# worxli/ORB_SLAM

Hardware: AMD Instinct MI355X
Metric: frames/sec ORB extract+match (640x480, 1000 kp) (higher is better)
Workload: dtype u8

## Files before the change

### orb_slam_amd/__init__.py

```python
import ctypes
import os
from pathlib import Path

import numpy as np

_PKG = Path(__file__).resolve().parent
LIB_PATH = Path(os.environ.get("ORBX_LIBRARY", _PKG / "liborbx.so"))

ORBX_OK = 0
ERRORS = {-1: "ORBX_ERR_ARG", -2: "ORBX_ERR_HIP", -3: "ORBX_ERR_CAPACITY",
          -4: "ORBX_ERR_UNSUPPORTED", -5: "ORBX_ERR_NOMEM", -6: "ORBX_ERR_NOT_POSDEF"}

KEYPOINT = np.dtype([("x", "<f4"), ("y", "<f4"), ("size", "<f4"), ("angle", "<f4"),
                     ("response", "<f4"), ("octave", "<i4"), ("class_id", "<i4")])
assert KEYPOINT.itemsize == 28


class OrbxError(RuntimeError):
    def __init__(self, code, where):
        super().__init__(f"{where}: {ERRORS.get(code, code)}")
        self.code = code


class FrameView(ctypes.Structure):
# ... 242 lines not shown
        "orbx_vocab_n_words": ([vp], i),
        "orbx_vocab_transform": ([vp, vp, i, vp, i, vp, vp, vp, vp, vp, ip, vp, vp, vp, ip], i),
        "orbx_dev_compute_bow": ([vp, vp, i, i, i], i),
        "orbx_dev_read_bow": ([vp, i, i, vp, vp, vp, vp, vp, ip, vp, vp, vp, ip], i),
        "orbx_dev_search_by_bow": ([vp, i, i, vp, f, i, vp, i, vp], i),
        "orbx_dev_search_by_bow_kf": ([vp, i, vp, i, vp, vp, f, i, vp, i, vp], i),
        "orbx_dev_search_for_triangulation": ([vp, i, vp, i, vp, vp, vp, vp, i, i, vp, i, vp], i),
        "orbx_undistort_keypoints": ([vp, i, vp, vp, vp, vp], i),
        "orbx_compute_image_bounds": ([i, i, vp, vp, vp], i),
        "orbx_dev_undistort": ([vp, i, i, vp, vp], i),
        "orbx_pose_optimization": ([vp, vp, ip, vp], i),
        "orbx_pose_optimization_batch": ([vp, i, vp, vp, vp], i),
        "orbx_pose_stage": ([vp, i, vp], i),
        "orbx_pose_run": ([vp], i),
        "orbx_pose_fetch": ([vp, vp, vp, vp], i),
        "orbx_version": ([], ctypes.c_char_p),
        "orbx_abi_version": ([], i),
        "orbx_lba_set_workgroups": ([vp, i], i),
        "orbx_lba_get_workgroups": ([vp], i),
        "orbx_lba_last_workgroups": ([vp], i),
        "orbx_debug_lba_split": ([vp, i, i, i, i], i),
        "orbx_debug_describe_patch": ([vp, i, i, i, i, vp], i),
        "orbx_debug_level0_direct": ([vp], i),
        "orbx_pose_set_exact": ([vp, i], i),
        "orbx_pose_get_exact": ([vp], i),
        "orbx_dev_set_image_bounds": ([vp, vp], i),
        "orbx_set_launch_mode": ([vp, i], i),
        "orbx_get_launch_mode": ([vp], i),
        "orbx_host_alloc": ([sz, ctypes.POINTER(vp)], i),
        "orbx_host_free": ([vp], None),
        "orbx_dev_upload_async": ([vp, i, i, vp, i, i, sz], i),
        "orbx_dev_download_async": ([vp, i, i, vp, vp, vp, vp, vp], i),
        "orbx_describe_levels": ([i, f, i, i, i, i, vp, i], i),
        "orbx_init_models": ([vp, vp], i),
        "orbx_init_models_batch": ([vp, i, vp], i),
        "orbx_dev_init_models": ([vp, i, i, i, f, i, vp], i),
        "orbx_dev_read_init_models": ([vp, i, vp], i),
        "orbx_init_reconstruct": ([vp, vp], i),
        "orbx_init_reconstruct_batch": ([vp, i, vp], i),
        "orbx_dev_init_reconstruct": ([vp, i, i, i, vp, f, f, i], i),
        "orbx_dev_read_init_reconstruct": ([vp, i, vp, ip], i),
        "orbx_triangulate_matches": ([vp, vp, i, vp, i, vp, vp, vp, vp, vp, vp, vp, vp], i),
        "orbx_create_new_map_points": ([vp, vp, vp, i, vp, vp, vp, i, i, vp, vp, vp, vp, vp, vp], i),
        "orbx_dev_create_new_map_points": ([vp, i, vp, vp, i, vp, vp, vp, vp, i, i, vp, vp, vp, vp, vp, vp, i], i),
    }
    for name, (args, res) in sigs.items():
# ... 150 lines not shown
        nm, n1 = ctypes.c_int(0), ctypes.c_int(0)
        _check(lib().orbx_dev_read_matches(self._h, slot, _ptr(m), self.nfeatures, ctypes.byref(nm),
                                           ctypes.byref(n1)), "orbx_dev_read_matches")
        return m, nm.value

    def level(self, slot, level, blurred=False, cap=4 << 20):
        buf = np.zeros(cap, np.uint8)
        pw, ph = ctypes.c_int(0), ctypes.c_int(0)
        _check(lib().orbx_dev_read_level(self._h, slot, level, int(blurred), _ptr(buf), cap,
                                         ctypes.byref(pw), ctypes.byref(ph)), "orbx_dev_read_level")
        return buf[:pw.value * ph.value].reshape(ph.value, pw.value).copy()

    def describe_patch(self, slot, level, x, y):
        out = np.zeros((37, 37), np.uint8)
        _check(lib().orbx_debug_describe_patch(self._h, slot, level, x, y, _ptr(out)), "orbx_debug_describe_patch")
        return out

    def level0_direct(self):
        r = lib().orbx_debug_level0_direct(self._h)
        if r < 0:
            raise OrbxError(r, "orbx_debug_level0_direct")
        return bool(r)

    def timing(self, enable=True, only=None):
        _check(lib().orbx_dev_kernel_time_select(self._h, only.encode() if only else None), "timing")
        _check(lib().orbx_dev_kernel_time_enable(self._h, int(enable)), "timing")

    def kernel_time(self, name):
        avg, tot = ctypes.c_double(0), ctypes.c_double(0)
        n = lib().orbx_dev_kernel_time(self._h, name.encode(), ctypes.byref(avg), ctypes.byref(tot))
        if n < 0:
            raise OrbxError(n, "orbx_dev_kernel_time")
        return n, avg.value, tot.value

    def pose_optimization(self, frames):
        from .synth_pose import PoseStats
        arr = (type(frames[0]) * len(frames))(*frames)
        n = np.zeros(len(frames), np.int32)
        st = (PoseStats * len(frames))()
        _check(lib().orbx_pose_optimization_batch(self._h, len(frames), arr, _ptr(n), st),
               "orbx_pose_optimization_batch")
        for k in range(len(frames)):
            frames[k].Tcw = arr[k].Tcw
        return n, list(st)

    def pose_stage(self, frames):
# ... 238 lines not shown
```

### orb_slam_amd/csrc/orbx_extract.hip

```cpp
#include <algorithm>
#include <type_traits>

#include "orbx_device.h"
#include "orbx_internal.h"

namespace orbx {

constexpr size_t kRetainLds = 128 * 1024;
constexpr int kRetainCellCap = 512;
constexpr int kSplitMinFrames = 16;
constexpr size_t kResizeLds = 96 * 1024;

__constant__ __attribute__((aligned(4))) int8_t c_pattern[256][4] = {
#include "orbx_pattern.inc"
};

#ifdef ORBX_FAST_PROFILE
__device__ unsigned long long g_fast_prof[16];
__device__ inline unsigned long long fp_stamp()
{
    unsigned long long t;
    asm volatile("s_memtime %0\n\ts_waitcnt lgkmcnt(0)" : "=s"(t)::"memory");
    return t;
}
#define FP_T0() unsigned long long _ft = fp_stamp()
#define FP_MARK(k)                                                                  \
    do {                                                                            \
        const unsigned long long _n = fp_stamp();                                   \
        if (threadIdx.x == 0) atomicAdd(&g_fast_prof[k], _n - _ft);                 \
        _ft = _n;                                                                   \
    } while (0)
#define FP_ADD(k, v) atomicAdd(&g_fast_prof[k], (unsigned long long)(v))
extern "C" int orbx_debug_fast_prof(unsigned long long* out)
{
    return hipMemcpyFromSymbol(out, HIP_SYMBOL(g_fast_prof), sizeof(unsigned long long) * 16) == hipSuccess ? 0 : -2;
}
#else
#define FP_T0()
#define FP_MARK(k)
#define FP_ADD(k, v)
#endif

struct ExtractArgs {
    const LevelGeom* levels;
    const CellGeom* cells;
    const ResizeCol* res_cols;
    const ResizeRow* res_rows;
    const int* umax;
    const uint8_t* frames;
    uint8_t* pyr_raw;
    uint8_t* pyr_blur;
    uint32_t* cell_lists;
    int32_t* cell_count;
    uint32_t* level_keys;
    int32_t* level_count;
    orbx_keypoint* out_kps;
    uint8_t* out_desc;
    int32_t* out_n;
// ... 19 lines not shown
    int stride;
};
static_assert(kEdge % 16 == 0, "the direct level 0 keeps the padded level's 16-byte alignment");
__device__ __forceinline__ LevelSrc level_src(const ExtractArgs& a, int f, int level, long long off, int stride)
{
    if (a.l0_direct && level == 0)
        return {a.frames + ((long long)(a.first_slot + f) * a.w * a.h - (long long)kEdge * a.w - kEdge), a.w};
    return {a.pyr_raw + (size_t)f * a.frame_pyr_bytes + off, stride};
}

template <class T>
__device__ __forceinline__ T cget(const T* p, int i)
{
#if defined(__HIP_DEVICE_COMPILE__)
    return ((const __attribute__((address_space(4))) T*)p)[i];
#else
    return p[i];
#endif
}

__device__ inline uint8_t sat_u8(int v) { return (uint8_t)min(max(v, 0), 255); }
__device__ inline int sat_s16(int v) { return min(max(v, -32768), 32767); }

struct RowWalk {
    int r, q, dr, dq, nq;
    __device__ RowWalk(int start, int stride, int n_q) : nq(n_q)
    {
        r = start / n_q;
        q = start - r * n_q;
        dr = stride / n_q;
        dq = stride - dr * n_q;
    }
    __device__ void next()
    {
        r += dr;
        q += dq;
        if (q >= nq) {
            q -= nq;
            r++;
        }
    }
};


template <int kBatch, typename T, typename Load>
__device__ inline void stage_to_lds(T* dst, int n, int tid, int nthr, Load load)
{
    for (int u0 = 0; u0 < n; u0 += kBatch * nthr) {
        T v[kBatch];
#pragma unroll
        for (int k = 0; k < kBatch; k++) v[k] = load(min(u0 + k * nthr + tid, n - 1));
#pragma unroll
        for (int k = 0; k < kBatch; k++) dst[min(u0 + k * nthr + tid, n - 1)] = v[k];
    }
}

constexpr int kPyrRows = 8;
constexpr int kPyr0Shift = (16 - kEdge % 16) % 16;

__global__ __launch_bounds__(256) void k_pyr_level0(ExtractArgs a, int q_lo, int nint)
{
    const int f = blockIdx.y;
    const LevelGeom L = cget(a.levels, 0);
    const int qpr = L.stride >> 4, nstrips = (L.ph + kPyrRows - 1) / kPyrRows;
    const int nbord = qpr - nint;
    int idx = blockIdx.x * blockDim.x + threadIdx.x;
    const uint8_t* src = a.frames + (size_t)(a.first_slot + f) * a.w * a.h;
// ... 515 lines not shown
                *reinterpret_cast<uint4*>(out + (size_t)(kEdge + r) * stride + 16 * q) =
                    *reinterpret_cast<const uint4*>(dst + (r - c0) * stride + 16 * q);
            }
            for (int i = tid; i < 2 * kEdge * n16; i += T) {
                const int k = i / n16, q = i - k * n16;
                const int py = k < kEdge ? k : L.h + k;
                const int r = reflect101(py - kEdge, L.h);
                if (r >= pl.x && r < pl.y)
                    *reinterpret_cast<uint4*>(out + (size_t)py * stride + 16 * q) =
                        *reinterpret_cast<const uint4*>(dst + (r - c0) * stride + 16 * q);
            }
        }
        CASC_MARK(l, 3);
        if (l > 0) {
            tcol += L.w;
            trow += max(0, nrows);
        }
        sc0 = c0;
        sstride = stride;
    }
}

typedef _Float16 orbx_h2 __attribute__((ext_vector_type(2)));
typedef unsigned short orbx_u16x2 __attribute__((ext_vector_type(2)));
__device__ inline orbx_h2 h2_min3(orbx_h2 a, orbx_h2 b, orbx_h2 c)
{
    return __builtin_elementwise_minimum(__builtin_elementwise_minimum(a, b), c);
}
__device__ inline orbx_h2 h2_max3(orbx_h2 a, orbx_h2 b, orbx_h2 c)
{
    return __builtin_elementwise_maximum(__builtin_elementwise_maximum(a, b), c);
}
__device__ inline void fast_arc2(const uint8_t* t, int pa, int pb, int pitch, int& Sa, int& Sb)
{
    const int off[16] = {3 * pitch,      1 + 3 * pitch, 2 + 2 * pitch,  3 + pitch,
                         3,              3 - pitch,     2 - 2 * pitch,  1 - 3 * pitch,
                         -3 * pitch,     -1 - 3 * pitch, -2 - 2 * pitch, -3 - pitch,
                         -3,             -3 + pitch,    -2 + 2 * pitch, -1 + 3 * pitch};
    const int o = 3 * pitch + 3;
    int ba = pa - o, bb = pb - o;
    asm("" : "+v"(ba), "+v"(bb));
    const uint8_t* ta = t + ba;
    const uint8_t* tb = t + bb;
    auto pair = [&](int k) {
        orbx_u16x2 pv;
        pv.x = ta[k];
        pv.y = tb[k];
        return __builtin_bit_cast(uint32_t, pv) | 0x64006400u;
    };
    const orbx_h2 v = __builtin_bit_cast(orbx_h2, pair(o));
    orbx_h2 d[16];
#pragma unroll
    for (int k = 0; k < 16; k++) {
        const uint32_t w = pair(off[k] + o);
        d[k] = v - __builtin_bit_cast(orbx_h2, w);
    }
    orbx_h2 lo3[16], hi3[16];
#pragma unroll
    for (int k = 0; k < 16; k++) {
        lo3[k] = h2_min3(d[k], d[(k + 1) & 15], d[(k + 2) & 15]);
        hi3[k] = h2_max3(d[k], d[(k + 1) & 15], d[(k + 2) & 15]);
    }
    orbx_h2 m9[16], x9[16];
#pragma unroll
    for (int k = 0; k < 16; k++) {
        m9[k] = h2_min3(lo3[k], lo3[(k + 3) & 15], lo3[(k + 6) & 15]);
        x9[k] = h2_max3(hi3[k], hi3[(k + 3) & 15], hi3[(k + 6) & 15]);
    }
    orbx_h2 dk = h2_max3(m9[0], m9[1], m9[2]), br = h2_min3(x9[0], x9[1], x9[2]);
#pragma unroll
    for (int k = 3; k < 15; k += 2) {
        dk = h2_max3(dk, m9[k], m9[k + 1]);
        br = h2_min3(br, x9[k], x9[k + 1]);
    }
    dk = __builtin_elementwise_maximum(dk, m9[15]);
    br = __builtin_elementwise_minimum(br, x9[15]);
    const orbx_h2 r = __builtin_elementwise_maximum(dk, -br);
    Sa = (int)(float)r.x;
    Sb = (int)(float)r.y;
}

__device__ inline int byte_of(uint32_t w, int k) { return (int)((w >> (8 * k)) & 0xFF); }

typedef short orbx_s16x2 __attribute__((ext_vector_type(2)));
__device__ inline uint32_t pk_sub16(uint32_t a, uint32_t b)
{
    return __builtin_bit_cast(uint32_t, (orbx_s16x2)(__builtin_bit_cast(orbx_s16x2, a) - __builtin_bit_cast(orbx_s16x2, b)));
}
__device__ inline uint32_t pk_max16(uint32_t a, uint32_t b)
{
    return __builtin_bit_cast(uint32_t,
                              __builtin_elementwise_max(__builtin_bit_cast(orbx_s16x2, a), __builtin_bit_cast(orbx_s16x2, b)));
}
__device__ inline orbx_h2 h2_bytes(uint32_t w, uint32_t k64, uint32_t sel)
{
    return __builtin_bit_cast(orbx_h2, __builtin_amdgcn_perm(k64, w, sel));
}

constexpr int kFastWideThreads = 256;
__host__ __device__ constexpr int fast_tile_bytes(int hy_max, int pitch) { return (hy_max * pitch + 511) & ~511; }
__host__ __device__ constexpr int fast_lds_bytes(int tile_bytes) { return 2 * tile_bytes + tile_bytes / 32; }
__host__ __device__ constexpr int fast_static_lds(bool u32_entries) { return 4 * 384 * (u32_entries ? 4 : 2) + 64; }
// ... 53 lines not shown
        const float inv16 = 1.0f / (float)nq16;
        auto row_of = [&](int i) { return (int)(((float)i + 0.5f) * inv16); };
        for (int u0 = 0; u0 < n; u0 += 4 * kBlock) {
            const int i0 = min(u0 + tid, n - 1), i1 = min(u0 + kBlock + tid, n - 1);
            const int i2 = min(u0 + 2 * kBlock + tid, n - 1), i3 = min(u0 + 3 * kBlock + tid, n - 1);
            const int r0 = row_of(i0), r1 = row_of(i1), r2 = row_of(i2), r3 = row_of(i3);
            const int c0 = i0 - r0 * nq16, c1 = i1 - r1 * nq16, c2 = i2 - r2 * nq16, c3 = i3 - r3 * nq16;
            const uint4 v0 = *reinterpret_cast<const uint4*>(src_w + (uint32_t)(r0 * lstride + 16 * c0));
            const uint4 v1 = *reinterpret_cast<const uint4*>(src_w + (uint32_t)(r1 * lstride + 16 * c1));
            const uint4 v2 = *reinterpret_cast<const uint4*>(src_w + (uint32_t)(r2 * lstride + 16 * c2));
            const uint4 v3 = *reinterpret_cast<const uint4*>(src_w + (uint32_t)(r3 * lstride + 16 * c3));
            t16[r0 * (P >> 4) + c0] = v0;
            t16[r1 * (P >> 4) + c1] = v1;
            t16[r2 * (P >> 4) + c2] = v2;
            t16[r3 * (P >> 4) + c3] = v3;
        }
    };
    auto clear_maps = [&]() { clear_maps_at(sm); };
    auto clear_kept = [&]() {
        for (int i = tid; i < (tile_bytes >> 7); i += kBlock) reinterpret_cast<uint4*>(kept)[i] = make_uint4(0, 0, 0, 0);
    };
    const int c_lo = 3 + sh, c_hi = hx - 4 + sh;
    const int q0 = c_lo >> 2, nqe = c_hi >= c_lo ? (c_hi >> 2) - q0 + 1 : 0;
    const int q_last = q0 + nqe - 1;
    const int j_lo = c_lo & 3, j_hi = c_hi & 3;
    const uint32_t k64 = 0x64646464u;
    auto score_pass = [&](const int tmin, const int sr0, const int nrows) {
        const int nunits = max(nrows, 0) * nqe;
        if (nunits <= 0) return;
        int qt = 0;
        auto set_nz = [&](int p) { atomicOr(&nz[p >> 7], 1u << ((p >> 2) & 31)); };
        auto score_pair = [&](int pa, int pb, bool has_a, bool has_b) {
            if (!has_a) return;
            int Sa, Sb;
            fast_arc2(tile, pa, pb, P, Sa, Sb);
            Sa -= 1;
            Sb -= 1;
            if (Sa >= tmin) {
                sm[pa] = (uint8_t)Sa;
                set_nz(pa);
            }
            if (has_b && Sb >= tmin) {
                sm[pb] = (uint8_t)Sb;
                set_nz(pb);
            }
        };
        const orbx_h2 T1 = {(_Float16)(tmin + 1), (_Float16)(tmin + 1)};
        RowWalk cw_(wv * 64 + lane, kBlock, nqe);
        for (int u0 = wv * 64; u0 < nunits; u0 += kBlock, cw_.next()) {
            const int u = u0 + lane;
            const int r = sr0 + cw_.r, q = q0 + cw_.q;
            uint32_t xw0 = 0xBC00BC00u, xw1 = 0xBC00BC00u;
            if (u < nunits) {
                const uint32_t* row = tile32 + r * nq + q;
                const uint32_t mid = row[0];
                const uint32_t lo = row[-1], hi = row[1];
                const uint32_t up = row[-3 * nq], dn = row[3 * nq];
                const uint32_t p4w = __builtin_amdgcn_alignbyte(hi, mid, 3);
                const uint32_t p12w = __builtin_amdgcn_alignbyte(mid, lo, 1);
                uint32_t xw[2];
#pragma unroll
                for (int hf = 0; hf < 2; hf++) {
                    const uint32_t sel = hf ? 0x04030401u : 0x04020400u;
                    const orbx_h2 v = h2_bytes(mid, k64, sel);
                    const orbx_h2 p0 = h2_bytes(dn, k64, sel), p4 = h2_bytes(p4w, k64, sel);
                    const orbx_h2 p8 = h2_bytes(up, k64, sel), p12 = h2_bytes(p12w, k64, sel);
                    const orbx_h2 A = __builtin_elementwise_maximum(__builtin_elementwise_minimum(p4, p12),
                                                                    __builtin_elementwise_minimum(p0, p8));
                    const orbx_h2 B = __builtin_elementwise_minimum(__builtin_elementwise_maximum(p4, p12),
                                                                    __builtin_elementwise_maximum(p0, p8));
                    const orbx_h2 x = __builtin_elementwise_maximum(v - A, B - v) - T1;
                    xw[hf] = __builtin_bit_cast(uint32_t, x);
                }
                xw0 = xw[0];
                xw1 = xw[1];
            }
            const bool at_q0 = q == q0, at_ql = q == q_last;
            const bool cut0 = at_q0 & (j_lo > 0), cut1 = (at_q0 & (j_lo > 1)) | (at_ql & (j_hi < 1));
            const bool cut2 = (at_q0 & (j_lo > 2)) | (at_ql & (j_hi < 2)), cut3 = at_ql & (j_hi < 3);
            const bool ok0 = (__builtin_bit_cast(orbx_h2, xw0).x >= (_Float16)0) & !cut0;
            const bool ok1 = (__builtin_bit_cast(orbx_h2, xw1).x >= (_Float16)0) & !cut1;
            const bool ok2 = ((int32_t)xw0 >= 0) & !cut2, ok3 = ((int32_t)xw1 >= 0) & !cut3;
            const uint64_t b0 = __builtin_amdgcn_ballot_w64(ok0), b1 = __builtin_amdgcn_ballot_w64(ok1);
            const uint64_t b2 = __builtin_amdgcn_ballot_w64(ok2), b3 = __builtin_amdgcn_ballot_w64(ok3);
            const int n0 = __popcll(b0), n1 = __popcll(b1), n2 = __popcll(b2);
            const int ntot = n0 + n1 + n2 + __popcll(b3);
#ifdef ORBX_FAST_PROFILE
            if (lane == 0) FP_ADD(10 + (tmin < 10), ntot);
            if (lane == 0) FP_ADD(12, 1);
#endif
            const int pbase = r * P + 4 * q;
            auto slot = [&](uint64_t bm, int start) {
                return (int)__builtin_amdgcn_mbcnt_hi((uint32_t)(bm >> 32),
                                                      __builtin_amdgcn_mbcnt_lo((uint32_t)bm, (uint32_t)start));
            };
            if (ok0) cand[slot(b0, qt)] = (QEntry)pbase;
            if (ok1) cand[slot(b1, qt + n0)] = (QEntry)(pbase + 1);
            if (ok2) cand[slot(b2, qt + n0 + n1)] = (QEntry)(pbase + 2);
            if (ok3) cand[slot(b3, qt + n0 + n1 + n2)] = (QEntry)(pbase + 3);
            qt = __builtin_amdgcn_readfirstlane(qt + ntot);
            if (qt >= 128) {
                __builtin_amdgcn_fence(__ATOMIC_RELEASE, "wavefront");
                __builtin_amdgcn_wave_barrier();
                __builtin_amdgcn_fence(__ATOMIC_ACQUIRE, "wavefront");
                int qh = 0;
                for (; qt - qh >= 128; qh += 128)
                    score_pair(cand[qh + lane], cand[qh + 64 + lane], true, true);
                const int rest = qt - qh;
                const QEntry e0 = lane < rest ? cand[qh + lane] : (QEntry)0;
                const QEntry e1 = lane + 64 < rest ? cand[qh + 64 + lane] : (QEntry)0;
                __builtin_amdgcn_fence(__ATOMIC_RELEASE, "wavefront");
                __builtin_amdgcn_wave_barrier();
                __builtin_amdgcn_fence(__ATOMIC_ACQUIRE, "wavefront");
                if (lane < rest) cand[lane] = e0;
                if (lane + 64 < rest) cand[lane + 64] = e1;
                qt = __builtin_amdgcn_readfirstlane(rest);
            }
        }
        if (lane == 0) s_left[wv] = qt;
        __syncthreads();
        int pre[kWaves + 1];
        pre[0] = 0;
#pragma unroll
        for (int w = 0; w < kWaves; w++) pre[w + 1] = pre[w] + s_left[w];
        const int T = pre[kWaves];
        auto entry = [&](int g) {
            int w = 0;
#pragma unroll
            for (int k = 1; k < kWaves; k++) w += g >= pre[k];
            return (int)(reinterpret_cast<const QEntry*>(qbuf) + w * kQueue)[g - pre[w]];
        };
        for (int b0 = wv * 128; b0 < T; b0 += kWaves * 128) {
            const int ga = b0 + lane, gb = b0 + 64 + lane;
            score_pair(ga < T ? entry(ga) : 0, gb < T ? entry(gb) : 0, ga < T, gb < T);
        }
    };
    auto nms_pass = [&](const int rb0, const int rb1, const int wh) {
        int c1 = 0;
        const uint32_t FT = (uint32_t)max(a.fast_th, 1) * 0x00010001u;
        auto nms_unit = [&](int idx) {
            const int rw = idx / nq, q = idx - rw * nq;
            if (rw < rb0 || rw >= rb1) return;
            const uint32_t* m = sm32 + idx;
            const uint32_t mid = m[0];
            uint32_t nb[8];
            int k = 0;
#pragma unroll
            for (int dr = 0; dr < 3; dr++) {
                const uint32_t* mr = m + (dr - 1) * nq;
                const uint32_t lo = q > 0 ? mr[-1] : 0u, mm = mr[0], hi = q + 1 < nq ? mr[1] : 0u;
                nb[k++] = __builtin_amdgcn_alignbyte(mm, lo, 3);
                if (dr != 1) nb[k++] = mm;
                nb[k++] = __builtin_amdgcn_alignbyte(hi, mm, 1);
            }
            uint32_t bits = 0;
#pragma unroll
// ... 13 lines not shown
        const int nw = (wh * nq + 31) >> 5;
        const int pw = (nw + kBlock - 1) / kBlock;
        const int w0 = min(tid * pw, nw), w1 = min(w0 + pw, nw);
        int cnt = 0;
        for (int w = w0; w < w1; w++) cnt += __popc(nz[w]);
        int total;
        const int off0 = block_exclusive_scan(cnt, &total, bs, 1);
        for (int base = 0; base < total; base += kUnitCap) {
            if (base > 0) __syncthreads();
            if (cnt && off0 < base + kUnitCap && off0 + cnt > base) {
                int off = off0;
                for (int w = w0; w < w1; w++) {
                    uint32_t b = nz[w];
                    while (b) {
                        const int bit = __builtin_ctz(b);
                        b &= b - 1;
                        if (off >= base && off < base + kUnitCap) ulist[off - base] = (uint16_t)(32 * w + bit);
                        off++;
                    }
                }
            }
            __syncthreads();
            const int n = min(total - base, kUnitCap);
            for (int i = tid; i < n; i += kBlock) nms_unit((int)ulist[i]);
        }
        return c1;
    };
    uint32_t* out = a.cell_lists + (size_t)f * a.list_entries + C.list_off;
    auto compact = [&](const int t, const int tmin, const int w0, const int wh, const int out_base) {
        const int nkw = (wh * P + 31) >> 5;
        const int per = (nkw + kBlock - 1) / kBlock;
        const int ka = min(tid * per, nkw), kb = min(ka + per, nkw);
        const bool all_kept = t == tmin;
        int cnt = 0;
        for (int k = ka; k < kb; k++) {
            uint32_t b = kept[k];
            if (all_kept) {
                cnt += __popc(b);
            } else {
                while (b) {
                    const int bit = __builtin_ctz(b);
                    b &= b - 1;
                    cnt += sm[32 * k + bit] >= t;
                }
            }
        }
        int total;
        int off = out_base + block_exclusive_scan(cnt, &total, bs, 1);
        if (cnt) {
            for (int k = ka; k < kb; k++) {
                uint32_t b = kept[k];
                while (b) {
                    const int bit = __builtin_ctz(b);
                    b &= b - 1;
                    const int pos = 32 * k + bit;
                    const int s = sm[pos];
// ... 858 lines not shown
    if (x < kEdge || x >= L.w - kEdge || y < kEdge || y >= L.h - kEdge) return ORBX_ERR_ARG;
    ctx_enter(ctx);
    uint8_t* d = nullptr;
    if (hipDeviceSynchronize() != hipSuccess) return ORBX_ERR_HIP;
    if (hipMalloc(&d, kBrRows * kBrRows) != hipSuccess) return ORBX_ERR_NOMEM;
    const bool direct = level == 0 && kEdge == 16 && ctx->geom.w % 16 == 0;
    const long long fw = ctx->geom.w, fh = ctx->geom.h;
    const uint8_t* lev = direct ? ctx->frames + ((long long)slot * fw * fh - (long long)kEdge * fw - kEdge)
                                : ctx->pyr_raw + (size_t)slot * ctx->geom.frame_pyr_bytes + L.off;
    hipLaunchKernelGGL(k_debug_describe_patch, dim3(1), dim3(64), 0, ctx->stream, lev, direct ? (int)fw : L.stride,
                       direct ? 1 : 0, L, kEdge + x, kEdge + y, d);
    int r = ORBX_OK;
    if (hipStreamSynchronize(ctx->stream) != hipSuccess ||
        hipMemcpy(out, d, kBrRows * kBrRows, hipMemcpyDeviceToHost) != hipSuccess)
        r = ORBX_ERR_HIP;
    (void)hipFree(d);
    return r;
}

extern "C" int orbx_debug_level0_direct(orbx_ctx* ctx)
{
    if (!ctx) return ORBX_ERR_ARG;
    return ctx->last_l0_direct ? 1 : 0;
}

namespace orbx {

int launch_extract(orbx_ctx* ctx, int first, int count, const MatchSpec* m)
{
    const Geometry& g = ctx->geom;
    if (count > 1 || (m && m->kind != 0 && ctx->async_match)) {
        const int r = ensure_aux_streams(ctx);
        if (r != ORBX_OK) return r;
    }
    for (int sl = first; sl < first + count && sl < (int)ctx->bow_ready.size(); sl++) ctx->bow_ready[sl] = 0;
    wait_uploads_overlap(ctx, first, count, ctx->stream);
    ExtractArgs a;
    a.levels = ctx->dgeom.levels;
    a.cells = ctx->dgeom.cells;
    a.res_cols = ctx->dgeom.res_cols;
    a.res_rows = ctx->dgeom.res_rows;
    a.umax = ctx->dgeom.umax;
    a.frames = ctx->frames;
    a.pyr_raw = ctx->pyr_raw + (size_t)first * g.frame_pyr_bytes;
    a.pyr_blur = nullptr;
    a.cell_lists = ctx->cell_lists + (size_t)first * g.list_entries;
// ... 87 lines not shown
    };
    auto run_rest = [&](const ExtractArgs& x, int nb, hipStream_t st, int parts) {
        if (parts & 1) {
        timer_begin(ctx, "fast", st);
        {
            int wmax = 0, hmax = 0;
            for (const CellGeom& c : g.cells) {
                if (!c.valid) continue;
                wmax = std::max(wmax, (15 + c.hx + 15) & ~15);
                hmax = std::max(hmax, c.hy);
            }
            const dim3 grid((int)g.cells.size(), nb);
            auto plan = [&](int P, int static_lds, int& band_rows) {
                band_rows = 0;
                const int whole = fast_tile_bytes(hmax, P);
                if (fast_lds_bytes(whole) + static_lds <= kFastLdsTarget || hmax <= 9) return whole;
                int wh = hmax;
                while (wh > 9 && fast_lds_bytes(fast_tile_bytes(wh, P)) + static_lds > kFastLdsTarget) wh--;
                const int nint = hmax - 6, bmax = wh - 8;
                const int nbands = (nint + bmax - 1) / bmax;
                band_rows = (nint + nbands - 1) / nbands;
                return fast_tile_bytes(std::min(hmax, band_rows + 8), P);
            };
            auto fast = [&](auto kern, int bytes, int band_rows, int threads) {
                const int lds = fast_lds_bytes(bytes);
                hipLaunchKernelGGL(kern, grid, dim3(threads), lds, st, x, bytes, band_rows);
            };
            int br = 0, bytes = 0;
            auto fits = [&](int P) {
                if (wmax > P) return false;
                bytes = fast_tile_bytes(hmax, P);
                return bytes <= 65536;
            };
            auto fits_banded = [&](int P) {
                if (wmax > P) return false;
                bytes = plan(P, fast_static_lds(false), br);
                return bytes <= 65536;
            };
            if (fits(96)) fast(k_fast_cells<96>, bytes, 0, 256);
            else if (fits(144)) {
                for (int rep = 0; rep < kDiagRepeat[3]; rep++) fast(k_fast_cells<144>, bytes, 0, 256);
            } else if (fits(208)) fast(k_fast_cells<208>, bytes, 0, 256);
            else if (fits_banded(336)) fast(k_fast_cells<336, kFastWideThreads, true>, bytes, br, kFastWideThreads);
            else {
                bytes = plan(wmax, fast_static_lds(true), br);
                fast(k_fast_cells<0, kFastWideThreads, true>, bytes, br, kFastWideThreads);
            }
        }
        timer_end(ctx, "fast", st);
        }
        if (parts & 2) {
        timer_begin(ctx, "retain", st);
        {
            const int ew = x.harris ? 2 : 1;
            const int cw = (ew + 1) * kRetainCellCap + 8;
            const int cwaves = 4;
            const int lw = (ew + 1) * g.max_level_cap + 8;
            const int lwaves = 1;
            const dim3 cgrid(((int)g.cells.size() + cwaves - 1) / cwaves, nb), lgrid((g.nlevels + lwaves - 1) / lwaves, nb);
            if (x.harris) {
                hipLaunchKernelGGL(k_harris_cells, dim3((int)g.cells.size(), nb), dim3(256), 0, st, x);
                hipLaunchKernelGGL(k_retain_cells<uint64_t>, cgrid, dim3(64 * cwaves), (size_t)cwaves * cw * 4, st, x,
                                   cwaves, cw);
                hipLaunchKernelGGL(k_retain_levels<uint64_t>, lgrid, dim3(64 * lwaves), (size_t)lwaves * lw * 4, st, x,
                                   lwaves, lw);
            } else {
                hipLaunchKernelGGL(k_retain_cells<uint32_t>, cgrid, dim3(64 * cwaves), (size_t)cwaves * cw * 4, st, x,
                                   cwaves, cw);
                hipLaunchKernelGGL(k_retain_levels<uint32_t>, lgrid, dim3(64 * lwaves), (size_t)lwaves * lw * 4, st, x,
// ... 132 lines not shown
```

### orb_slam_amd/csrc/orbx_internal.h

```cpp
#pragma once

#include <hip/hip_runtime.h>

#include <cstdint>
#include <memory>
#include <string>
#include <vector>

#include "../../include/orbx.h"

namespace orbx {

constexpr int kEdge = 16;
constexpr int kHalfPatch = 15;
constexpr int kPatch = 31;
constexpr int kMaxLevels = 16;
constexpr int kMaxFeatures = 4096;
constexpr int kGridCols = 64;
constexpr int kGridRows = 48;
#ifndef ORBX_BLUR_STRIP
#define ORBX_BLUR_STRIP 28
#endif
constexpr int kBlurStrip = ORBX_BLUR_STRIP;
constexpr int kBlurItems = 256;
// ... 166 lines not shown
    uint64_t* level_keys64 = nullptr;
    int harris = 0;
    int fp_contract = 0;
    int nth_pivot = ORBX_NTH_PIVOT_GCC48;
    int32_t* level_count = nullptr;
    orbx_keypoint* out_kps = nullptr;
    uint8_t* out_desc = nullptr;
    int32_t* out_n = nullptr;
    int32_t* match12 = nullptr;
    int32_t* match_n = nullptr;
    int32_t* error_flags = nullptr;
    long long cap_frame_px = 0;
    long long cap_pyr_bytes = 0;
    long long cap_list_entries = 0;
    long long cap_level_entries = 0;
    int cap_cells = 0;
    int cap_res_cols = 0, cap_res_rows = 0, cap_blur_tiles = 0;
    int4* blur_tiles = nullptr;
    int4* cascade = nullptr;
    int cap_cascade = 0;
    int blur_tiles_n = 0;
    int last_first = 0, last_count = 0;
    bool last_l0_direct = false;
    int has_bounds = 0;
    float bounds[4] = {0.f, 0.f, 0.f, 0.f};
    void* scratch = nullptr;
    size_t scratch_bytes = 0;
    void* host_pinned = nullptr;
    size_t host_pinned_bytes = 0;
    orbx::LbaResident* lba_res = nullptr;
    int lba_workgroups = 0;
    void* lba_split = nullptr;
    size_t lba_split_bytes = 0;
    int lba_split_cap[2] = {0, 0};
    size_t lba_split_cap_lds[2] = {0, 0};
    int lba_last_workgroups = 0;
    bool lba_force_single = false;
    bool lba_split_timed_out = false;
    bool lba_split_fallback = true;
    int lba_split_coop = 0;
    int lba_dbg_fail = 0;
    int lba_dbg_cap = 0;
    int lba_res_iters[2] = {0, 0};
    void* pose_dev = nullptr;
    size_t pose_dev_bytes = 0;
    void* pose_host = nullptr;
// ... 114 lines not shown
```

Baseline: 294,700.

## Streamline FAST arc scoring and candidate compaction with scalar-mask LDS writes

Rewrites the FAST arc-score network to build on pairwise min/max of adjacent ring differences, so fewer min3/max3 operations are needed. It also drops the 0x6400 half-float bias trick in favour of raw byte bit-casts, and returns both packed scores as one word. The candidate scan replaces the RowWalk integer walk with incremental pointer stepping and precomputed scalar cut masks. Candidate entries are written to LDS with inline asm that switches the exec mask per ballot, and the tail iteration is peeled. The change also adds debug entry points and profiling counters; the risks are correctness of the half-precision denormal path and fragile hand-written exec manipulation.

Measured after the change: 304,900 (median of 6 runs). +3.5%, better.

```diff
diff --git a/orb_slam_amd/__init__.py b/orb_slam_amd/__init__.py
--- a/orb_slam_amd/__init__.py
+++ b/orb_slam_amd/__init__.py
@@ -288,6 +288,8 @@
         "orbx_debug_lba_split": ([vp, i, i, i, i], i),
         "orbx_debug_describe_patch": ([vp, i, i, i, i, vp], i),
         "orbx_debug_level0_direct": ([vp], i),
+        "orbx_debug_fast_instance": ([vp, vp], i),
+        "orbx_debug_fast_lists": ([vp, i, vp, i, vp, i, vp], i),
         "orbx_pose_set_exact": ([vp, i], i),
         "orbx_pose_get_exact": ([vp], i),
         "orbx_dev_set_image_bounds": ([vp, vp], i),
@@ -484,6 +486,26 @@
             raise OrbxError(r, "orbx_debug_level0_direct")
         return bool(r)
 
+    def fast_instance(self):
+        out = np.zeros(3, np.int32)
+        _check(lib().orbx_debug_fast_instance(self._h, _ptr(out)), "orbx_debug_fast_instance")
+        return tuple(int(v) for v in out)
+
+    def fast_lists(self, slot, cells_cap=1 << 14, lists_cap=1 << 22):
+        cells = np.zeros(10 * cells_cap, np.int32)
+        lists = np.zeros(lists_cap, np.uint32)
+        ne = ctypes.c_int(0)
+        n = lib().orbx_debug_fast_lists(self._h, slot, _ptr(cells), cells.size, _ptr(lists), lists.size,
+                                        ctypes.byref(ne))
+        _check(min(n, 0), "orbx_debug_fast_lists")
+        out = []
+        for level, ini_x, ini_y, hx, hy, valid, off, cap, cnt, _ in cells[:10 * n].reshape(n, 10):
+            assert 0 <= cnt <= cap and off + cnt <= ne.value, (cnt, cap, off, ne.value)
+            e = lists[off:off + cnt]
+            xy = np.stack([e & 0xFFF, (e >> 12) & 0xFFF, e >> 24], axis=1).astype(np.int64)
+            out.append((int(level), int(ini_x), int(ini_y), int(hx), int(hy), bool(valid), xy))
+        return out
+
     def timing(self, enable=True, only=None):
         _check(lib().orbx_dev_kernel_time_select(self._h, only.encode() if only else None), "timing")
         _check(lib().orbx_dev_kernel_time_enable(self._h, int(enable)), "timing")
diff --git a/orb_slam_amd/csrc/orbx_extract.hip b/orb_slam_amd/csrc/orbx_extract.hip
--- a/orb_slam_amd/csrc/orbx_extract.hip
+++ b/orb_slam_amd/csrc/orbx_extract.hip
@@ -16,7 +16,7 @@
 };
 
 #ifdef ORBX_FAST_PROFILE
-__device__ unsigned long long g_fast_prof[16];
+__device__ unsigned long long g_fast_prof[24];
 __device__ inline unsigned long long fp_stamp()
 {
     unsigned long long t;
@@ -33,7 +33,7 @@
 #define FP_ADD(k, v) atomicAdd(&g_fast_prof[k], (unsigned long long)(v))
 extern "C" int orbx_debug_fast_prof(unsigned long long* out)
 {
-    return hipMemcpyFromSymbol(out, HIP_SYMBOL(g_fast_prof), sizeof(unsigned long long) * 16) == hipSuccess ? 0 : -2;
+    return hipMemcpyFromSymbol(out, HIP_SYMBOL(g_fast_prof), sizeof(unsigned long long) * 24) == hipSuccess ? 0 : -2;
 }
 #else
 #define FP_T0()
@@ -99,27 +99,6 @@
 __device__ inline uint8_t sat_u8(int v) { return (uint8_t)min(max(v, 0), 255); }
 __device__ inline int sat_s16(int v) { return min(max(v, -32768), 32767); }
 
-struct RowWalk {
-    int r, q, dr, dq, nq;
-    __device__ RowWalk(int start, int stride, int n_q) : nq(n_q)
-    {
-        r = start / n_q;
-        q = start - r * n_q;
-        dr = stride / n_q;
-        dq = stride - dr * n_q;
-    }
-    __device__ void next()
-    {
-        r += dr;
-        q += dq;
-        if (q >= nq) {
-            q -= nq;
-            r++;
-        }
-    }
-};
-
-
 template <int kBatch, typename T, typename Load>
 __device__ inline void stage_to_lds(T* dst, int n, int tid, int nthr, Load load)
 {
@@ -681,7 +660,6 @@
 }
 
 typedef _Float16 orbx_h2 __attribute__((ext_vector_type(2)));
-typedef unsigned short orbx_u16x2 __attribute__((ext_vector_type(2)));
 __device__ inline orbx_h2 h2_min3(orbx_h2 a, orbx_h2 b, orbx_h2 c)
 {
     return __builtin_elementwise_minimum(__builtin_elementwise_minimum(a, b), c);
@@ -690,7 +668,7 @@
 {
     return __builtin_elementwise_maximum(__builtin_elementwise_maximum(a, b), c);
 }
-__device__ inline void fast_arc2(const uint8_t* t, int pa, int pb, int pitch, int& Sa, int& Sb)
+__device__ inline uint32_t fast_arc2(const uint8_t* t, int pa, int pb, int pitch)
 {
     const int off[16] = {3 * pitch,      1 + 3 * pitch, 2 + 2 * pitch,  3 + pitch,
                          3,              3 - pitch,     2 - 2 * pitch,  1 - 3 * pitch,
@@ -701,42 +679,34 @@
     asm("" : "+v"(ba), "+v"(bb));
     const uint8_t* ta = t + ba;
     const uint8_t* tb = t + bb;
-    auto pair = [&](int k) {
-        orbx_u16x2 pv;
-        pv.x = ta[k];
-        pv.y = tb[k];
-        return __builtin_bit_cast(uint32_t, pv) | 0x64006400u;
-    };
-    const orbx_h2 v = __builtin_bit_cast(orbx_h2, pair(o));
+    auto pair = [&](int k) { return __builtin_bit_cast(orbx_h2, (uint32_t)ta[k] | ((uint32_t)tb[k] << 16)); };
+    const orbx_h2 v = pair(o);
     orbx_h2 d[16];
 #pragma unroll
-    for (int k = 0; k < 16; k++) {
-        const uint32_t w = pair(off[k] + o);
-        d[k] = v - __builtin_bit_cast(orbx_h2, w);
-    }
-    orbx_h2 lo3[16], hi3[16];
-#pragma unroll
-    for (int k = 0; k < 16; k++) {
-        lo3[k] = h2_min3(d[k], d[(k + 1) & 15], d[(k + 2) & 15]);
-        hi3[k] = h2_max3(d[k], d[(k + 1) & 15], d[(k + 2) & 15]);
-    }
-    orbx_h2 m9[16], x9[16];
-#pragma unroll
-    for (int k = 0; k < 16; k++) {
-        m9[k] = h2_min3(lo3[k], lo3[(k + 3) & 15], lo3[(k + 6) & 15]);
-        x9[k] = h2_max3(hi3[k], hi3[(k + 3) & 15], hi3[(k + 6) & 15]);
-    }
-    orbx_h2 dk = h2_max3(m9[0], m9[1], m9[2]), br = h2_min3(x9[0], x9[1], x9[2]);
-#pragma unroll
-    for (int k = 3; k < 15; k += 2) {
-        dk = h2_max3(dk, m9[k], m9[k + 1]);
-        br = h2_min3(br, x9[k], x9[k + 1]);
-    }
-    dk = __builtin_elementwise_maximum(dk, m9[15]);
-    br = __builtin_elementwise_minimum(br, x9[15]);
-    const orbx_h2 r = __builtin_elementwise_maximum(dk, -br);
-    Sa = (int)(float)r.x;
-    Sb = (int)(float)r.y;
+    for (int k = 0; k < 16; k++) d[k] = v - pair(off[k] + o);
+    orbx_h2 qn[8], qx[8];
+#pragma unroll
+    for (int j = 0; j < 8; j++) {
+        qn[j] = __builtin_elementwise_minimum(d[2 * j + 1], d[(2 * j + 2) & 15]);
+        qx[j] = __builtin_elementwise_maximum(d[2 * j + 1], d[(2 * j + 2) & 15]);
+    }
+    orbx_h2 m[8], x[8];
+#pragma unroll
+    for (int j = 0; j < 8; j++) {
+        const orbx_h2 e0 = d[2 * j], e9 = d[(2 * j + 9) & 15];
+        m[j] = h2_min3(h2_min3(qn[j], qn[(j + 1) & 7], qn[(j + 2) & 7]), qn[(j + 3) & 7],
+                       __builtin_elementwise_maximum(e0, e9));
+        x[j] = h2_max3(h2_max3(qx[j], qx[(j + 1) & 7], qx[(j + 2) & 7]), qx[(j + 3) & 7],
+                       __builtin_elementwise_minimum(e0, e9));
+    }
+    orbx_h2 dk = h2_max3(m[0], m[1], m[2]), br = h2_min3(x[0], x[1], x[2]);
+    dk = h2_max3(dk, m[3], m[4]);
+    br = h2_min3(br, x[3], x[4]);
+    dk = h2_max3(dk, m[5], m[6]);
+    br = h2_min3(br, x[5], x[6]);
+    dk = __builtin_elementwise_maximum(dk, m[7]);
+    br = __builtin_elementwise_minimum(br, x[7]);
+    return __builtin_bit_cast(uint32_t, __builtin_elementwise_maximum(dk, -br));
 }
 
 __device__ inline int byte_of(uint32_t w, int k) { return (int)((w >> (8 * k)) & 0xFF); }
@@ -836,20 +806,16 @@
     };
     const int c_lo = 3 + sh, c_hi = hx - 4 + sh;
     const int q0 = c_lo >> 2, nqe = c_hi >= c_lo ? (c_hi >> 2) - q0 + 1 : 0;
-    const int q_last = q0 + nqe - 1;
     const int j_lo = c_lo & 3, j_hi = c_hi & 3;
     const uint32_t k64 = 0x64646464u;
     auto score_pass = [&](const int tmin, const int sr0, const int nrows) {
         const int nunits = max(nrows, 0) * nqe;
         if (nunits <= 0) return;
-        int qt = 0;
         auto set_nz = [&](int p) { atomicOr(&nz[p >> 7], 1u << ((p >> 2) & 31)); };
         auto score_pair = [&](int pa, int pb, bool has_a, bool has_b) {
             if (!has_a) return;
-            int Sa, Sb;
-            fast_arc2(tile, pa, pb, P, Sa, Sb);
-            Sa -= 1;
-            Sb -= 1;
+            const uint32_t rb = fast_arc2(tile, pa, pb, P);
+            const int Sa = (int)(int16_t)rb - 1, Sb = ((int32_t)rb >> 16) - 1;
             if (Sa >= tmin) {
                 sm[pa] = (uint8_t)Sa;
                 set_nz(pa);
@@ -860,66 +826,112 @@
             }
         };
         const orbx_h2 T1 = {(_Float16)(tmin + 1), (_Float16)(tmin + 1)};
-        RowWalk cw_(wv * 64 + lane, kBlock, nqe);
-        for (int u0 = wv * 64; u0 < nunits; u0 += kBlock, cw_.next()) {
-            const int u = u0 + lane;
-            const int r = sr0 + cw_.r, q = q0 + cw_.q;
-            uint32_t xw0 = 0xBC00BC00u, xw1 = 0xBC00BC00u;
-            if (u < nunits) {
-                const uint32_t* row = tile32 + r * nq + q;
-                const uint32_t mid = row[0];
-                const uint32_t lo = row[-1], hi = row[1];
-                const uint32_t up = row[-3 * nq], dn = row[3 * nq];
-                const uint32_t p4w = __builtin_amdgcn_alignbyte(hi, mid, 3);
-                const uint32_t p12w = __builtin_amdgcn_alignbyte(mid, lo, 1);
-                uint32_t xw[2];
-#pragma unroll
-                for (int hf = 0; hf < 2; hf++) {
-                    const uint32_t sel = hf ? 0x04030401u : 0x04020400u;
-                    const orbx_h2 v = h2_bytes(mid, k64, sel);
-                    const orbx_h2 p0 = h2_bytes(dn, k64, sel), p4 = h2_bytes(p4w, k64, sel);
-                    const orbx_h2 p8 = h2_bytes(up, k64, sel), p12 = h2_bytes(p12w, k64, sel);
-                    const orbx_h2 A = __builtin_elementwise_maximum(__builtin_elementwise_minimum(p4, p12),
-                                                                    __builtin_elementwise_minimum(p0, p8));
-                    const orbx_h2 B = __builtin_elementwise_minimum(__builtin_elementwise_maximum(p4, p12),
-                                                                    __builtin_elementwise_maximum(p0, p8));
-                    const orbx_h2 x = __builtin_elementwise_maximum(v - A, B - v) - T1;
-                    xw[hf] = __builtin_bit_cast(uint32_t, x);
-                }
-                xw0 = xw[0];
-                xw1 = xw[1];
-            }
-            const bool at_q0 = q == q0, at_ql = q == q_last;
-            const bool cut0 = at_q0 & (j_lo > 0), cut1 = (at_q0 & (j_lo > 1)) | (at_ql & (j_hi < 1));
-            const bool cut2 = (at_q0 & (j_lo > 2)) | (at_ql & (j_hi < 2)), cut3 = at_ql & (j_hi < 3);
-            const bool ok0 = (__builtin_bit_cast(orbx_h2, xw0).x >= (_Float16)0) & !cut0;
-            const bool ok1 = (__builtin_bit_cast(orbx_h2, xw1).x >= (_Float16)0) & !cut1;
-            const bool ok2 = ((int32_t)xw0 >= 0) & !cut2, ok3 = ((int32_t)xw1 >= 0) & !cut3;
-            const uint64_t b0 = __builtin_amdgcn_ballot_w64(ok0), b1 = __builtin_amdgcn_ballot_w64(ok1);
-            const uint64_t b2 = __builtin_amdgcn_ballot_w64(ok2), b3 = __builtin_amdgcn_ballot_w64(ok3);
-            const int n0 = __popcll(b0), n1 = __popcll(b1), n2 = __popcll(b2);
-            const int ntot = n0 + n1 + n2 + __popcll(b3);
+        auto cut_mask = [](bool c) {
+            const uint32_t m = __builtin_amdgcn_readfirstlane(c ? ~0u : 0u);
+            uint64_t r = ((uint64_t)m << 32) | m;
+            asm("" : "+s"(r));
+            return r;
+        };
+        const uint64_t cutA0 = cut_mask(j_lo > 0), cutA1 = cut_mask(j_lo > 1), cutA2 = cut_mask(j_lo > 2);
+        const uint64_t cutB1 = cut_mask(j_hi < 1), cutB2 = cut_mask(j_hi < 2), cutB3 = cut_mask(j_hi < 3);
+        typedef __attribute__((address_space(3))) QEntry LdsEntry;
+        const uint32_t cand_lds = __builtin_amdgcn_readfirstlane((uint32_t)(uintptr_t)(LdsEntry*)cand);
+        constexpr int kEsh = sizeof(QEntry) == 2 ? 1 : 2;
+        uint32_t qe = cand_lds;
+        auto compass = [&](const int pos, const int qr, const uint64_t live) {
+            const uint32_t* row = reinterpret_cast<const uint32_t*>(tile + pos);
+            const uint32_t mid = row[0];
+            const uint32_t lo = row[-1], hi = row[1];
+            const uint32_t up = row[-3 * nq], dn = row[3 * nq];
+            const uint32_t p4w = __builtin_amdgcn_alignbyte(hi, mid, 3);
+            const uint32_t p12w = __builtin_amdgcn_alignbyte(mid, lo, 1);
+            uint32_t xw[2];
+#pragma unroll
+            for (int hf = 0; hf < 2; hf++) {
+                const uint32_t sel = hf ? 0x04030401u : 0x04020400u;
+                const orbx_h2 v = h2_bytes(mid, k64, sel);
+                const orbx_h2 p0 = h2_bytes(dn, k64, sel), p4 = h2_bytes(p4w, k64, sel);
+                const orbx_h2 p8 = h2_bytes(up, k64, sel), p12 = h2_bytes(p12w, k64, sel);
+                const orbx_h2 A = __builtin_elementwise_maximum(__builtin_elementwise_minimum(p4, p12),
+                                                                __builtin_elementwise_minimum(p0, p8));
+                const orbx_h2 B = __builtin_elementwise_minimum(__builtin_elementwise_maximum(p4, p12),
+                                                                __builtin_elementwise_maximum(p0, p8));
+                const orbx_h2 x = __builtin_elementwise_maximum(v - A, B - v) - T1;
+                xw[hf] = __builtin_bit_cast(uint32_t, x);
+            }
+            const uint64_t at0 = __builtin_amdgcn_ballot_w64(qr == 0), atl = __builtin_amdgcn_ballot_w64(qr == nqe - 1);
+            const uint64_t b0 = __builtin_amdgcn_ballot_w64(__builtin_bit_cast(orbx_h2, xw[0]).x >= (_Float16)0) &
+                                ~(at0 & cutA0) & live;
+            const uint64_t b1 = __builtin_amdgcn_ballot_w64(__builtin_bit_cast(orbx_h2, xw[1]).x >= (_Float16)0) &
+                                ~((at0 & cutA1) | (atl & cutB1)) & live;
+            const uint64_t b2 = __builtin_amdgcn_ballot_w64((int32_t)xw[0] >= 0) & ~((at0 & cutA2) | (atl & cutB2)) & live;
+            const uint64_t b3 = __builtin_amdgcn_ballot_w64((int32_t)xw[1] >= 0) & ~(atl & cutB3) & live;
+            const int n0 = __popcll(b0), n1 = __popcll(b1), n2 = __popcll(b2), n3 = __popcll(b3);
+            auto slot = [&](uint64_t bm, uint32_t base) {
+                asm("" : "+s"(base));
+                const uint32_t rank = __builtin_amdgcn_mbcnt_hi((uint32_t)(bm >> 32), __builtin_amdgcn_mbcnt_lo((uint32_t)bm, 0u));
+                return (rank << kEsh) + base;
+            };
+            const uint32_t s1 = qe + ((uint32_t)n0 << kEsh), s2 = s1 + ((uint32_t)n1 << kEsh);
+            const uint32_t s3 = s2 + ((uint32_t)n2 << kEsh);
+            const uint32_t a0 = slot(b0, qe), a1 = slot(b1, s1), a2 = slot(b2, s2), a3 = slot(b3, s3);
+            const uint32_t e0 = (uint32_t)pos, e1 = e0 | 1u, e2 = e0 | 2u, e3 = e0 | 3u;
+            uint64_t saved;
+            if constexpr (sizeof(QEntry) == 2)
+                asm volatile("s_mov_b64 %0, exec\n\t"
+                             "s_mov_b64 exec, %1\n\tds_write_b16 %5, %9\n\t"
+                             "s_mov_b64 exec, %2\n\tds_write_b16 %6, %10\n\t"
+                             "s_mov_b64 exec, %3\n\tds_write_b16 %7, %11\n\t"
+                             "s_mov_b64 exec, %4\n\tds_write_b16 %8, %12\n\t"
+                             "s_mov_b64 exec, %0"
+                             : "=&s"(saved)
+                             : "s"(b0), "s"(b1), "s"(b2), "s"(b3), "v"(a0), "v"(a1), "v"(a2), "v"(a3), "v"(e0), "v"(e1),
+                               "v"(e2), "v"(e3)
+                             : "memory");
+            else
+                asm volatile("s_mov_b64 %0, exec\n\t"
+                             "s_mov_b64 exec, %1\n\tds_write_b32 %5, %9\n\t"
+                             "s_mov_b64 exec, %2\n\tds_write_b32 %6, %10\n\t"
+                             "s_mov_b64 exec, %3\n\tds_write_b32 %7, %11\n\t"
+                             "s_mov_b64 exec, %4\n\tds_write_b32 %8, %12\n\t"
+                             "s_mov_b64 exec, %0"
+                             : "=&s"(saved)
+                             : "s"(b0), "s"(b1), "s"(b2), "s"(b3), "v"(a0), "v"(a1), "v"(a2), "v"(a3), "v"(e0), "v"(e1),
+                               "v"(e2), "v"(e3)
+                             : "memory");
+            qe = __builtin_amdgcn_readfirstlane(s3 + ((uint32_t)n3 << kEsh));
 #ifdef ORBX_FAST_PROFILE
-            if (lane == 0) FP_ADD(10 + (tmin < 10), ntot);
+            if (lane == 0) FP_ADD(10 + (tmin < 10), n0 + n1 + n2 + n3);
             if (lane == 0) FP_ADD(12, 1);
 #endif
-            const int pbase = r * P + 4 * q;
-            auto slot = [&](uint64_t bm, int start) {
-                return (int)__builtin_amdgcn_mbcnt_hi((uint32_t)(bm >> 32),
-                                                      __builtin_amdgcn_mbcnt_lo((uint32_t)bm, (uint32_t)start));
-            };
-            if (ok0) cand[slot(b0, qt)] = (QEntry)pbase;
-            if (ok1) cand[slot(b1, qt + n0)] = (QEntry)(pbase + 1);
-            if (ok2) cand[slot(b2, qt + n0 + n1)] = (QEntry)(pbase + 2);
-            if (ok3) cand[slot(b3, qt + n0 + n1 + n2)] = (QEntry)(pbase + 3);
-            qt = __builtin_amdgcn_readfirstlane(qt + ntot);
-            if (qt >= 128) {
+        };
+        const int wvu = __builtin_amdgcn_readfirstlane(wv);
+        const int start = wvu * 64 + lane, row0 = start / nqe;
+        uint32_t qr = start - row0 * nqe;
+        int pos = 4 * ((sr0 + row0) * nq + q0 + (int)qr);
+        const int dr = kBlock / nqe, dq = kBlock - dr * nqe;
+        const int step = 4 * (dr * nq + dq);
+        int wrap_pos = 4 * (nq - nqe);
+        asm("" : "+v"(wrap_pos));
+        int u0 = wvu * 64;
+        for (; u0 + 64 <= nunits; u0 += kBlock) {
+            compass(pos, (int)qr, ~0ull);
+            qr += dq;
+            const uint32_t qw = qr - (uint32_t)nqe;
+            pos += step + ((int32_t)qw >= 0 ? wrap_pos : 0);
+            qr = min(qr, qw);
+            if (qe - cand_lds >= (128u << kEsh)) {
+                const int qt = (int)((qe - cand_lds) >> kEsh);
                 __builtin_amdgcn_fence(__ATOMIC_RELEASE, "wavefront");
                 __builtin_amdgcn_wave_barrier();
                 __builtin_amdgcn_fence(__ATOMIC_ACQUIRE, "wavefront");
                 int qh = 0;
-                for (; qt - qh >= 128; qh += 128)
+                for (; qt - qh >= 128; qh += 128) {
+#ifdef ORBX_FAST_PROFILE
+                    if (lane == 0) FP_ADD(13, 1);
+#endif
                     score_pair(cand[qh + lane], cand[qh + 64 + lane], true, true);
+                }
                 const int rest = qt - qh;
                 const QEntry e0 = lane < rest ? cand[qh + lane] : (QEntry)0;
                 const QEntry e1 = lane + 64 < rest ? cand[qh + 64 + lane] : (QEntry)0;
@@ -928,10 +940,15 @@
                 __builtin_amdgcn_fence(__ATOMIC_ACQUIRE, "wavefront");
                 if (lane < rest) cand[lane] = e0;
                 if (lane + 64 < rest) cand[lane + 64] = e1;
-                qt = __builtin_amdgcn_readfirstlane(rest);
-            }
-        }
-        if (lane == 0) s_left[wv] = qt;
+                qe = cand_lds + ((uint32_t)__builtin_amdgcn_readfirstlane(rest) << kEsh);
+            }
+        }
+        if (u0 < nunits) {
+            const int rem = nunits - u0;
+            const int pos0 = __builtin_amdgcn_readfirstlane(pos);
+            compass(lane < rem ? pos : pos0, (int)qr, (1ull << rem) - 1);
+        }
+        if (lane == 0) s_left[wv] = (int)((qe - cand_lds) >> kEsh);
         __syncthreads();
         int pre[kWaves + 1];
         pre[0] = 0;
@@ -946,6 +963,10 @@
         };
         for (int b0 = wv * 128; b0 < T; b0 += kWaves * 128) {
             const int ga = b0 + lane, gb = b0 + 64 + lane;
+#ifdef ORBX_FAST_PROFILE
+            if (lane == 0) FP_ADD(14, 1);
+            if (lane == 0) FP_ADD(15, min(128, T - b0));
+#endif
             score_pair(ga < T ? entry(ga) : 0, gb < T ? entry(gb) : 0, ga < T, gb < T);
         }
     };
@@ -1005,6 +1026,10 @@
             }
             __syncthreads();
             const int n = min(total - base, kUnitCap);
+#ifdef ORBX_FAST_PROFILE
+            if (tid == 0) FP_ADD(16, n);
+            if (tid == 0) FP_ADD(17, (n + kBlock - 1) / kBlock);
+#endif
             for (int i = tid; i < n; i += kBlock) nms_unit((int)ulist[i]);
         }
         return c1;
@@ -1015,6 +1040,9 @@
         const int per = (nkw + kBlock - 1) / kBlock;
         const int ka = min(tid * per, nkw), kb = min(ka + per, nkw);
         const bool all_kept = t == tmin;
+#ifdef ORBX_FAST_PROFILE
+        if (tid == 0) FP_ADD(18, per);
+#endif
         int cnt = 0;
         for (int k = ka; k < kb; k++) {
             uint32_t b = kept[k];
@@ -1919,6 +1947,37 @@
 {
     if (!ctx) return ORBX_ERR_ARG;
     return ctx->last_l0_direct ? 1 : 0;
+}
+
+extern "C" int orbx_debug_fast_instance(orbx_ctx* ctx, int* out)
+{
+    if (!ctx || !out || ctx->last_fast[0] < 0) return ORBX_ERR_ARG;
+    for (int k = 0; k < 3; k++) out[k] = ctx->last_fast[k];
+    return ORBX_OK;
+}
+
+extern "C" int orbx_debug_fast_lists(orbx_ctx* ctx, int slot, int32_t* cells, int cells_cap, uint32_t* lists,
+                                     int lists_cap, int* entries)
+{
+    using namespace orbx;
+    if (!ctx || !cells || !lists || !entries || slot < 0 || slot >= ctx->slots) return ORBX_ERR_ARG;
+    ctx_enter(ctx);
+    const Geometry& g = ctx->geom;
+    const int n = (int)g.cells.size();
+    if (cells_cap < 10 * n || lists_cap < g.list_entries) return ORBX_ERR_CAPACITY;
+    std::vector<int32_t> cnt(n);
+    if (hipDeviceSynchronize() != hipSuccess ||
+        hipMemcpy(cnt.data(), ctx->cell_count + (size_t)slot * n, 4 * (size_t)n, hipMemcpyDeviceToHost) != hipSuccess ||
+        hipMemcpy(lists, ctx->cell_lists + (size_t)slot * g.list_entries, 4 * (size_t)g.list_entries,
+                  hipMemcpyDeviceToHost) != hipSuccess)
+        return ORBX_ERR_HIP;
+    for (int c = 0; c < n; c++) {
+        const CellGeom& C = g.cells[c];
+        const int32_t v[10] = {C.level, C.ini_x, C.ini_y, C.hx, C.hy, C.valid ? 1 : 0, C.list_off, C.list_cap, cnt[c], 0};
+        for (int k = 0; k < 10; k++) cells[10 * c + k] = v[k];
+    }
+    *entries = g.list_entries;
+    return n;
 }
 
 namespace orbx {
@@ -2052,8 +2111,11 @@
                 band_rows = (nint + nbands - 1) / nbands;
                 return fast_tile_bytes(std::min(hmax, band_rows + 8), P);
             };
-            auto fast = [&](auto kern, int bytes, int band_rows, int threads) {
+            auto fast = [&](auto kern, int pitch, int bytes, int band_rows, int threads) {
                 const int lds = fast_lds_bytes(bytes);
+                ctx->last_fast[0] = pitch;
+                ctx->last_fast[1] = threads;
+                ctx->last_fast[2] = band_rows;
                 hipLaunchKernelGGL(kern, grid, dim3(threads), lds, st, x, bytes, band_rows);
             };
             int br = 0, bytes = 0;
@@ -2067,14 +2129,15 @@
                 bytes = plan(P, fast_static_lds(false), br);
                 return bytes <= 65536;
             };
-            if (fits(96)) fast(k_fast_cells<96>, bytes, 0, 256);
+            if (fits(96)) fast(k_fast_cells<96>, 96, bytes, 0, 256);
             else if (fits(144)) {
-                for (int rep = 0; rep < kDiagRepeat[3]; rep++) fast(k_fast_cells<144>, bytes, 0, 256);
-            } else if (fits(208)) fast(k_fast_cells<208>, bytes, 0, 256);
-            else if (fits_banded(336)) fast(k_fast_cells<336, kFastWideThreads, true>, bytes, br, kFastWideThreads);
+                for (int rep = 0; rep < kDiagRepeat[3]; rep++) fast(k_fast_cells<144>, 144, bytes, 0, 256);
+            } else if (fits(208)) fast(k_fast_cells<208>, 208, bytes, 0, 256);
+            else if (fits_banded(336))
+                fast(k_fast_cells<336, kFastWideThreads, true>, 336, bytes, br, kFastWideThreads);
             else {
                 bytes = plan(wmax, fast_static_lds(true), br);
-                fast(k_fast_cells<0, kFastWideThreads, true>, bytes, br, kFastWideThreads);
+                fast(k_fast_cells<0, kFastWideThreads, true>, 0, bytes, br, kFastWideThreads);
             }
         }
         timer_end(ctx, "fast", st);
diff --git a/orb_slam_amd/csrc/orbx_internal.h b/orb_slam_amd/csrc/orbx_internal.h
--- a/orb_slam_amd/csrc/orbx_internal.h
+++ b/orb_slam_amd/csrc/orbx_internal.h
@@ -212,6 +212,7 @@
     int blur_tiles_n = 0;
     int last_first = 0, last_count = 0;
     bool last_l0_direct = false;
+    int last_fast[3] = {-1, 0, 0};
     int has_bounds = 0;
     float bounds[4] = {0.f, 0.f, 0.f, 0.f};
     void* scratch = nullptr;
```
